# szaguldo-kamaz/FRI-ReinforcementLearning-C

Measured on AMD Instinct MI355X. Metric: rule-distance evals/sec (rules x envs), higher is better.
Workload: dtype f64; 1 GPU; cfg4_acrobot_64k_x_8k_per_gpu; nant=5, universe_len=41, rules_per_env=65536, envs_per_gpu=8192, exact_hits=4, dist_backend=none, world_size=1

## Files before the change

fri-reinforcementlearning-c_amd/__init__.py:

```python
import ctypes as C
import os

PKG_DIR = os.path.dirname(os.path.abspath(__file__))
ROOT = os.path.dirname(PKG_DIR)
HIP_LIB_PATH = os.environ.get("FRIRL_HIP_LIB_OVERRIDE") or os.path.join(PKG_DIR, "lib", "libfrirl_hip.so")

NO_HIT = 0xFFFFFFFF
MAX_NANT = 16
MAX_ACTIONS = 32


class FrirlHipError(RuntimeError):
    pass


class Tables(C.Structure):
    _fields_ = [("nant", C.c_int32), ("U", C.c_int32), ("u", C.c_void_p), ("ve", C.c_void_p)]


class RuleBases(C.Structure):
    _fields_ = [("E", C.c_int32), ("maxR", C.c_int32), ("rb", C.c_void_p), ("nrules", C.c_void_p), ("uidx", C.c_void_p)]


MAX_GRID = 64
# ... 71 lines not shown
    "frirl_hip_pack_codes": (C.c_int, [C.POINTER(Tables), C.POINTER(RuleBases), C.c_void_p, C.POINTER(C.c_int32), C.c_void_p, C.c_void_p]),
    "five_hip_rule_distance_coded_ws": (C.c_int, [C.POINTER(Tables), C.POINTER(RuleBases), C.c_void_p, C.c_void_p, C.POINTER(C.c_int32), C.c_void_p,
                                                  C.c_void_p, C.c_void_p, C.c_void_p, C.c_void_p, C.c_size_t, C.c_void_p]),
    "five_hip_sqrt_unscaled_check": (C.c_int, [C.c_void_p, C.c_void_p, C.c_void_p, C.c_int64, C.c_void_p]),
    "five_hip_rule_distance_sq_guard": (C.c_int, [C.POINTER(Tables), C.c_int32, C.c_void_p, C.c_void_p, C.c_void_p]),
    "five_hip_vag_concl": (C.c_int, [C.POINTER(Tables), C.POINTER(RuleBases), C.c_int, C.c_void_p, C.c_void_p, C.c_void_p, C.c_void_p]),
    "five_hip_vag_concl_weight": (C.c_int, [C.POINTER(Tables), C.POINTER(RuleBases), C.c_int, C.c_void_p, C.c_void_p, C.c_void_p, C.c_void_p]),
    "frirl_hip_get_best_action": (C.c_int, [C.POINTER(Tables), C.POINTER(RuleBases), C.c_int, C.c_void_p, C.c_void_p, C.c_int,
                                            C.c_void_p, C.c_void_p, C.c_void_p]),
    "five_hip_shepard_weight_check": (C.c_int, [C.c_void_p, C.c_int64, C.c_int, C.c_int, C.c_void_p, C.c_void_p]),
    "frirl_hip_explore_check": (C.c_int, [C.POINTER(AgentDesc), C.c_int64, C.c_void_p, C.c_void_p, C.c_void_p, C.c_void_p, C.c_void_p, C.c_void_p,
                                          C.c_void_p]),
    "five_hip_vag_concl_shared": (C.c_int, [C.POINTER(Tables), C.POINTER(RuleBases), C.c_int, C.c_int32, C.c_void_p, C.c_void_p, C.c_void_p, C.c_void_p]),
    "frirl_hip_get_best_action_shared": (C.c_int, [C.POINTER(Tables), C.POINTER(RuleBases), C.c_int, C.c_int32, C.c_void_p, C.c_void_p, C.c_int,
                                                   C.c_void_p, C.c_void_p, C.c_void_p]),
    "frirl_hip_rollout_shared": (C.c_int, [C.POINTER(Tables), C.POINTER(RuleBases), C.POINTER(AgentDesc), C.c_int32, C.POINTER(RolloutDesc), C.c_void_p]),
    "frirl_hip_reduce_shared": (C.c_int, [C.POINTER(Tables), C.POINTER(RuleBases), C.POINTER(AgentDesc), C.c_void_p, C.c_int, C.c_double, C.c_int,
                                          C.POINTER(C.c_int32), C.POINTER(ReduceResult), C.c_void_p]),
    "frirl_hip_lanes_preferred": (C.c_int, [C.c_int32, C.c_int32, C.c_int32]),
    "frirl_hip_lanes_workspace_bytes": (C.c_size_t, [C.c_int32, C.c_int32, C.c_int32, C.c_int32]),
    "frirl_hip_episode_run_lanes": (C.c_int, [C.POINTER(Tables), C.POINTER(RuleBases), C.POINTER(AgentDesc), C.POINTER(EnvsDesc), C.c_int32,
                                              C.c_void_p, C.c_size_t, C.c_void_p]),
    "frirl_hip_rollout_resident_rules": (C.c_int, [C.c_int32, C.c_int32, C.c_int32, C.c_int32]),
    "frirl_hip_learn_supported": (C.c_int, [C.c_int32, C.c_int32, C.c_int32, C.c_int32, C.c_int32]),
    "frirl_hip_learn_plan": (C.c_int, [C.c_int32, C.c_int32, C.POINTER(C.c_int32), C.POINTER(C.c_int32)]),
    "frirl_hip_learn_workspace_bytes": (C.c_size_t, [C.c_int32, C.c_int32, C.c_int32, C.c_int32]),
    "frirl_hip_learn_run": (C.c_int, [C.POINTER(Tables), C.POINTER(RuleBases), C.POINTER(AgentDesc), C.POINTER(EnvsDesc), C.POINTER(ConvergenceDesc),
                                      C.c_void_p, C.c_int32, C.c_int32, C.c_int32, C.c_void_p, C.c_void_p, C.c_void_p, C.c_size_t, C.c_void_p]),
    "frirl_hip_learn_train_workspace_bytes": (C.c_size_t, [C.c_int32, C.c_int32, C.c_int32, C.c_int32]),
    "frirl_hip_learn_train": (C.c_int, [C.POINTER(Tables), C.POINTER(RuleBases), C.POINTER(AgentDesc), C.POINTER(EnvsDesc), C.POINTER(ConvergenceDesc),
                                        C.c_int32, C.c_int32, C.c_void_p, C.c_void_p, C.c_void_p, C.c_void_p, C.c_size_t, C.POINTER(C.c_int32),
                                        LEARN_CHUNK_FN, C.c_void_p, C.c_void_p]),
    "five_hip_add_rule": (C.c_int, [C.POINTER(Tables), C.POINTER(RuleBases), C.c_void_p, C.c_void_p, C.c_void_p, C.c_void_p, C.c_void_p,
                                    C.c_void_p]),
    "frirl_hip_update_sarsa": (C.c_int, [C.POINTER(Tables), C.POINTER(RuleBases), C.POINTER(AgentDesc), C.POINTER(EnvsDesc), C.c_void_p,
                                         C.c_void_p, C.c_void_p, C.c_void_p, C.c_void_p]),
    "frirl_hip_env_step": (C.c_int, [C.POINTER(AgentDesc), C.c_int32, C.c_int32, C.c_void_p, C.c_void_p, C.c_void_p, C.c_void_p, C.c_void_p,
                                     C.c_void_p, C.c_void_p]),
    "frirl_hip_episode_begin": (C.c_int, [C.POINTER(Tables), C.POINTER(RuleBases), C.POINTER(AgentDesc), C.POINTER(EnvsDesc), C.c_void_p]),
    "frirl_hip_episode_step": (C.c_int, [C.POINTER(Tables), C.POINTER(RuleBases), C.POINTER(AgentDesc), C.POINTER(EnvsDesc), C.c_void_p]),
    "frirl_hip_episode_steps": (C.c_int, [C.POINTER(Tables), C.POINTER(RuleBases), C.POINTER(AgentDesc), C.POINTER(EnvsDesc), C.c_int32, C.c_void_p]),
    "frirl_hip_agent_begin": (C.c_int, [C.POINTER(Tables), C.POINTER(RuleBases), C.POINTER(AgentDesc), C.POINTER(EnvsDesc), C.POINTER(AgentIO), C.c_void_p]),
    "frirl_hip_agent_observe": (C.c_int, [C.POINTER(Tables), C.POINTER(RuleBases), C.POINTER(AgentDesc), C.POINTER(EnvsDesc), C.POINTER(AgentIO),
                                          C.c_void_p]),
    "frirl_hip_policy_begin": (C.c_int, [C.POINTER(Tables), C.POINTER(RuleBases), C.POINTER(AgentDesc), C.POINTER(PolicyRowsDesc), C.POINTER(AgentIO), C.c_void_p]),
    "frirl_hip_policy_observe": (C.c_int, [C.POINTER(Tables), C.POINTER(RuleBases), C.POINTER(AgentDesc), C.POINTER(PolicyRowsDesc), C.POINTER(AgentIO),
# ... 74 lines not shown
        for name, (res, args) in SIGNATURES.items():
            fn = getattr(L, name)
            fn.restype, fn.argtypes = res, args
        _lib = L
    return _lib


def check(rc, what=""):
    if rc != 0:
        raise FrirlHipError(f"{what}: rc={rc}: {lib().frirl_hip_last_error().decode()}")


def set_option(name, value):
    old = C.c_int()
    check(lib().frirl_hip_get_option(name.encode(), C.byref(old)), "frirl_hip_get_option")
    check(lib().frirl_hip_set_option(name.encode(), int(value)), "frirl_hip_set_option")
    return old.value


def _ptr(t):
    return None if t is None else C.c_void_p(t.data_ptr())


def _stream(stream=None):
    import torch
    s = stream if stream is not None else torch.cuda.current_stream()
    return C.c_void_p(s.cuda_stream)


class Problem:

    def __init__(self, u, ve, rb, nrules, uidx=None):
        import torch
        assert u.is_cuda and ve.is_cuda and rb.is_cuda and nrules.is_cuda
        assert u.dtype == torch.float64 and ve.dtype == torch.float64 and rb.dtype == torch.float64 and nrules.dtype == torch.int32
        self.nant, self.U = u.shape
        self.E, cols, self.maxR = rb.shape
        assert cols == self.nant + 1 and ve.shape == u.shape and nrules.shape == (self.E,)
        self.u, self.ve, self.rb, self.nrules = u.contiguous(), ve.contiguous(), rb.contiguous(), nrules.contiguous()
        self.uidx = None
        if uidx is not None:
            assert uidx.is_cuda and uidx.dtype == torch.int16 and uidx.shape == (self.E, self.nant, self.maxR) and self.U <= 32767
            self.uidx = uidx.contiguous()
        self.tables = Tables(self.nant, self.U, self.u.data_ptr(), self.ve.data_ptr())
        self._bases = RuleBases(self.E, self.maxR, self.rb.data_ptr(), self.nrules.data_ptr(),
                                self.uidx.data_ptr() if self.uidx is not None else None)
# ... 631 lines not shown
    for k in range(nant):
        idx = torch.randint(0, U, (E, R), generator=g, device=device)
        if k == nant - 1:
            idx = a_idx[torch.randint(0, A, (E, R), generator=g, device=device)]
        gk = d["grids"][k]
        lo_i, hi_i = int(np.argmin(np.abs(d["u"][k] - gk.min()))), int(np.argmin(np.abs(d["u"][k] - gk.max())))
        divider = ncorner >> (k + 1)
        corner = torch.tensor([lo_i if ((j // divider) % 2) == 0 else hi_i for j in range(ncorner)], device=device)
        idx[:, :ncorner] = corner[None]
        rb[:, k, :R] = ve_d[k][idx]
        if keep_rant:
            rant[:, k, :R] = u_d[k][idx]
        if compressed:
            uidx[:, k, :R] = idx.to(torch.int16)
        del idx
    rb[:, nant, ncorner:R] = torch.rand((E, R - ncorner), generator=g, device=device, dtype=torch.float64) * 3000.0 - 1500.0
    nrules = torch.full((E,), R, dtype=torch.int32, device=device)
    prob = Problem(u_d, ve_d, rb, nrules, uidx)
    agent = demo_agent(d, device, max_steps)
    envs = Envs(prob, device, keep_rant=keep_rant, rant_init=rant)
    return prob, agent, envs


def demo_agent(d, device, max_steps=None, p=0, **kw):
    return Agent(device, d["nant"], d["grids"], d["grid_div"], d["values_def"], d["action_ve"], d["alpha"], d["gamma"], d["qdiff_pos"],
                 d["qdiff_neg"], d["weight_thr"], d["skip_rules"], p, d["kind"], max_steps or d["max_steps"],
                 reward_good_above=d["reward_good_above"], qdiff_final_tolerance=d["qdiff_final_tolerance"], **kw)


def describe(states, actions, U, alpha, gamma, qdiff_pos, qdiff_neg, weight_thr=0.05, skip_rules=1, reward_good_above=0.0,
             qdiff_final_tolerance=250.0, max_steps=1000, name="external"):
    import numpy as np
    D = dropin()
    dims = list(states) + [dict(actions, steep=0.0, default=0.0)]
    nant = len(dims)
    assert 2 <= nant <= MAX_NANT - 1
    grid = np.zeros((nant, MAX_GRID))
    grid_len = np.zeros(nant, dtype=np.int32)
    grid_div, values_def, steep, udiv = np.zeros(nant), np.zeros(nant), np.zeros(nant), np.zeros(nant)
    for k, d in enumerate(dims):
        if d.get("values") is not None:
            v = np.asarray(d["values"], dtype=np.float64)
        else:
            v = np.zeros(int(d["n"]))
            D.frirl_gen_fixres_arr(v.ctypes.data_as(C.POINTER(C.c_double)), len(v), float(d["div"]))
        assert 1 <= len(v) <= MAX_GRID
# ... 43 lines not shown
```

fri-reinforcementlearning-c_amd/csrc/device_common.h:

```cpp
#pragma once

#include <hip/hip_runtime.h>
#include <stdint.h>

#include "../../include/frirl_hip.h"

#define FRIRL_WAVE 64
#define FRIRL_BLOCK 256
#define FRIRL_WAVES_PER_BLOCK (FRIRL_BLOCK / FRIRL_WAVE)

namespace frirl {

__device__ __forceinline__ unsigned snap_index(const double *__restrict__ uni, int len, double point, double div)
{
    const int low = (int)((point - uni[0]) / div);
    if (low < 0) return 0u;
    if (low >= len) return (unsigned)(len - 1);
    if (low + 1 >= len) return (unsigned)low;
    const double d1 = uni[low] - point;
    const double d2 = uni[low + 1] - point;
    return (fabs(d1) <= fabs(d2)) ? (unsigned)low : (unsigned)(low + 1);
}

__device__ __forceinline__ double universe_div(const double *__restrict__ uni, int U)
{
    return (uni[U - 1] - uni[0]) / (double)(U - 1);
}

__device__ __forceinline__ double observe_ve(const double *__restrict__ u, const double *__restrict__ ve, int U, int k, double xk)
{
    const double *uni = u + (size_t)k * U;
    return ve[(size_t)k * U + snap_index(uni, U, xk, universe_div(uni, U))];
}

#ifndef FRIRL_DECODE_MAD
#define FRIRL_DECODE_MAD 1
#endif
typedef __attribute__((address_space(3))) const double lds_cdouble;
__device__ __forceinline__ double2 lds_table_pair(const double *tab_k, uint32_t w)
{
    double2 v;
#if FRIRL_DECODE_MAD
    const uint32_t base = (uint32_t)(uintptr_t)(lds_cdouble *)tab_k;
    uint32_t a0, a1;
    asm("v_mad_u32_u16 %0, %1, 8, %2 op_sel:[0,0,0,0]" : "=v"(a0) : "v"(w), "s"(base));
    asm("v_mad_u32_u16 %0, %1, 8, %2 op_sel:[1,0,0,0]" : "=v"(a1) : "v"(w), "s"(base));
    v.x = *(lds_cdouble *)(uintptr_t)a0;
// ... 87 lines not shown

struct Options {
    int no_uidx;
    int rd_unroll;
    int rd_chunk;
    int rd_nt;
    int rd_persist;
    int rd_order;
    int rd_packed;
    int rd_sqdiff;
    int rd_qpass;
    int rd_prepass;
    int rd_coded;
    int step_wave;
    int step_track;
    int lanes_slices;
    int lanes_wpe;
    int rollout_group;
    int rollout_slices;
    int rollout_resident;
    int rollout_cap;
    int rollout_pair;
    int rollout_wps;
    int policy_group;
    int policy_slices;
    int learn_slices;
    int learn_alone;
    int learn_persistent;
    int multi_loopback;
    int mirror_sync;
    int no_many;
};
const Options &opts();
}
```

fri-reinforcementlearning-c_amd/csrc/rollout.hip:

```cpp
#include "sweeps.h"
#include "envs.h"
#include <mutex>
#include <type_traits>
#include <vector>

namespace frirl {

constexpr int RR_BLOCK = 256;

struct RolloutCtl {
    unsigned next[32];
    unsigned count[8];
    unsigned too_big;
    unsigned pad[7];
};

struct RolloutPark {
    int32_t *env;
    double *states;
    double *total;
    int32_t *steps;
    int32_t *act;
};

struct RolloutPhase {
    int from_parked;
    int stage;
    unsigned lo, hi;
    int cap;
    int qslot;
    int rps;
    int ht;
};

constexpr uint32_t HT_EMPTY = 0xFFFFFFFFu;

__device__ __forceinline__ uint32_t hash_mix(uint32_t hsh, double x)
// ... 455 lines not shown
            const PairSpec<NANT> &o = spec_s[buf][act_s[buf]];
#pragma unroll
            for (int k = 0; k < NS; k++) { states[k] = o.state[k]; q[k] = o.q[k]; }
            total = total + o.reward;
            success = o.success;
            steps++;
            fresh = false;
            ended = success == 1 || steps >= ag.max_steps;
        }
        if (threadIdx.x == 0) {
            ro.steps[qi] = steps;
            ro.reward[qi] = total;
            if (ro.success) ro.success[qi] = success;
            if (ro.final_states)
                for (int k = 0; k < NS; k++) ro.final_states[(size_t)qi * NS + k] = states[k];
            item_s = atomicAdd(&ctl->next[ph.qslot], 1u);
        }
        __syncthreads();
        item = (unsigned)__builtin_amdgcn_readfirstlane((int)item_s);
        __syncthreads();
    }
}

}

using namespace frirl_host;

namespace {

struct StreamWs { hipStream_t s; int dev; char *p; size_t bytes; };
std::mutex g_ws_mu;
std::vector<StreamWs> g_ws;
struct WsCleanup { ~WsCleanup() { for (StreamWs &w : g_ws) if (w.p) (void)hipFree(w.p); } } g_ws_cleanup;
char *stream_workspace(hipStream_t s, size_t bytes)
{
    int dev = 0;
    (void)hipGetDevice(&dev);
    std::lock_guard<std::mutex> lk(g_ws_mu);
    for (StreamWs &w : g_ws)
        if (w.s == s && w.dev == dev) {
            if (w.bytes >= bytes) return w.p;
            (void)hipStreamSynchronize(s);
            (void)hipFree(w.p);
            w.p = nullptr; w.bytes = 0;
            if (hipMalloc(reinterpret_cast<void **>(&w.p), bytes) != hipSuccess) { (void)hipGetLastError(); w.p = nullptr; return nullptr; }
            w.bytes = bytes;
            return w.p;
        }
    StreamWs w{s, dev, nullptr, bytes};
    if (hipMalloc(reinterpret_cast<void **>(&w.p), bytes) != hipSuccess) { (void)hipGetLastError(); return nullptr; }
    g_ws.push_back(w);
    return w.p;
}

int g_cus = 0;
int device_cus()
{
    if (g_cus) return g_cus;
    int dev = 0, n = 0;
    if (hipGetDevice(&dev) != hipSuccess || hipDeviceGetAttribute(&n, hipDeviceAttributeMultiprocessorCount, dev) != hipSuccess || n < 1) n = 256;
    g_cus = n;
    return n;
}

template <int N, int NA, int KIND, int H, bool EXCL>
void launch_phase(const frirl_hip_tables *t, const frirl_hip_rulebases *b, const frirl_hip_agent *ag, int Q, const frirl_hip_rollout *ro,
                  frirl::RolloutCtl *ctl, const frirl::RolloutPark &src, const frirl::RolloutPark &dst, const frirl::RolloutPhase &ph, unsigned items_max, int wps,
                  hipStream_t s)
{
    const size_t dyn = (size_t)(N + 1) * ph.rps * sizeof(double) + (KIND != FRIRL_HIP_ENV_CARTPOLE ? 2 * sizeof(double) * N * (size_t)t->U : 0) + sizeof(uint32_t) * (size_t)ph.ht +
                       (EXCL ? (size_t)ph.rps : 0);
    const long need = ((long)items_max * H + frirl::RR_BLOCK - 1) / frirl::RR_BLOCK;
// ... 131 lines not shown
        int H0 = 2;
        while (H0 < 64 && (long)Q * (2 * H0) <= lanes) H0 *= 2;
        if (o.rollout_slices == 2 || o.rollout_slices == 4 || o.rollout_slices == 8 || o.rollout_slices == 16 || o.rollout_slices == 32 || o.rollout_slices == 64) H0 = o.rollout_slices;
        ph.from_parked = 0; ph.stage = 0; ph.cap = nstages > 1 ? budget[0] : never;
        PHASE(H0, (unsigned)Q, list[0], list[0]);
        unsigned in_max = (unsigned)Q;
        for (int st = 1; st < nstages; st++) {
            ph.from_parked = 1; ph.stage = st; ph.cap = st == nstages - 1 ? never : budget[st];
            const frirl::RolloutPark &src = list[(st - 1) & 1], &dst = list[st & 1];
            for (int H = 64; H >= 2; H /= 2) {
                const long fit = lanes / H;
                ph.lo = H == 64 ? 0u : (unsigned)(fit / 2 < 0xffffffffL ? fit / 2 : 0xffffffffL);
                ph.hi = H == 2 ? 0xffffffffu : (unsigned)fit;
                if (ph.lo >= in_max) continue;
                PHASE(H, (unsigned)((long)in_max < fit || H == 2 ? in_max : fit), src, dst);
            }
        }
    }
#undef PHASE
    *too_big_flag = rps_full > cap_rules ? &ctl->too_big : nullptr;
    *workspace = nullptr;
    return 1;
}
```

fri-reinforcementlearning-c_amd/csrc/runtime.hip:

```cpp
#include <stdarg.h>
#include <stdio.h>
#include <stdlib.h>
#include <string.h>

#include <mutex>

#include "device_common.h"

namespace frirl_host {

static thread_local char g_err[512] = "";

void set_error(const char *fmt, ...)
{
    va_list ap;
    va_start(ap, fmt);
    vsnprintf(g_err, sizeof g_err, fmt, ap);
    va_end(ap);
}

static Options g_opts;
static std::once_flag g_opts_once;
struct OptName { const char *name, *env; int Options::*field; int def; };
static const OptName k_opts[] = {
    {"no_uidx", "FRIRL_HIP_NO_UIDX", &Options::no_uidx, 0},
    {"rd_unroll", "FRIRL_HIP_RD_UNROLL", &Options::rd_unroll, 0},
    {"rd_chunk", "FRIRL_HIP_RD_CHUNK", &Options::rd_chunk, 0},
    {"rd_nt", "FRIRL_HIP_RD_NT", &Options::rd_nt, -1},
    {"rd_persist", "FRIRL_HIP_RD_PERSIST", &Options::rd_persist, -1},
    {"rd_order", "FRIRL_HIP_RD_ORDER", &Options::rd_order, 0},
    {"rd_packed", "FRIRL_HIP_RD_PACKED", &Options::rd_packed, 1},
    {"rd_sqdiff", "FRIRL_HIP_RD_SQDIFF", &Options::rd_sqdiff, 1},
    {"rd_qpass", "FRIRL_HIP_RD_QPASS", &Options::rd_qpass, 0},
    {"rd_prepass", "FRIRL_HIP_RD_PREPASS", &Options::rd_prepass, 1},
    {"rd_coded", "FRIRL_HIP_RD_CODED", &Options::rd_coded, 1},
    {"step_wave", "FRIRL_HIP_STEP_WAVE", &Options::step_wave, -1},
    {"step_track", "FRIRL_HIP_STEP_TRACK", &Options::step_track, -1},
    {"lanes_slices", "FRIRL_HIP_LANES_SLICES", &Options::lanes_slices, 0},
    {"lanes_wpe", "FRIRL_HIP_LANES_WPE", &Options::lanes_wpe, 0},
    {"rollout_group", "FRIRL_HIP_ROLLOUT_GROUP", &Options::rollout_group, 0},
    {"rollout_slices", "FRIRL_HIP_ROLLOUT_SLICES", &Options::rollout_slices, 0},
    {"rollout_resident", "FRIRL_HIP_ROLLOUT_RESIDENT", &Options::rollout_resident, -1},
    {"rollout_cap", "FRIRL_HIP_ROLLOUT_CAP", &Options::rollout_cap, 0},
    {"rollout_pair", "FRIRL_HIP_ROLLOUT_PAIR", &Options::rollout_pair, -1},
    {"rollout_wps", "FRIRL_HIP_ROLLOUT_WPS", &Options::rollout_wps, 0},
    {"policy_group", "FRIRL_HIP_POLICY_GROUP", &Options::policy_group, 0},
    {"policy_slices", "FRIRL_HIP_POLICY_SLICES", &Options::policy_slices, 0},
    {"learn_slices", "FRIRL_HIP_LEARN_SLICES", &Options::learn_slices, 0},
    {"learn_alone", "FRIRL_HIP_LEARN_ALONE", &Options::learn_alone, 0},
    {"learn_persistent", "FRIRL_HIP_LEARN_PERSISTENT", &Options::learn_persistent, -1},
    {"multi_loopback", "FRIRL_HIP_MULTI_LOOPBACK", &Options::multi_loopback, 0},
    {"no_many", "FRIRL_HIP_NO_MANY", &Options::no_many, 0},
    {"mirror_sync", "FRIRL_HIP_MIRROR_SYNC", &Options::mirror_sync, 0},
};
static void opts_init()
{
    for (const OptName &o : k_opts) {
        const char *e = getenv(o.env);
        g_opts.*(o.field) = e ? atoi(e) : o.def;
    }
}
const Options &opts()
{
    std::call_once(g_opts_once, opts_init);
    return g_opts;
}
static const OptName *find_opt(const char *name)
{
// ... 104 lines not shown
```

fri-reinforcementlearning-c_amd/csrc/shared.hip:

```cpp
#include "shared_sweep.h"
#include "envs.h"
#include "reduce_plan.h"
#include <algorithm>
#include <cstdlib>
#include <cstring>
#include <cmath>
#include <numeric>
#include <vector>

namespace frirl {

template <int NANT, int AMAX, bool GBA>
__global__ __launch_bounds__(SH_BLOCK) void shared_q_kernel(const double *__restrict__ u, const double *__restrict__ ve, int U,
                                                             const double *__restrict__ rb, const int32_t *__restrict__ nrules, int maxR, int p,
                                                             int Q, const double *__restrict__ x, const double *__restrict__ action_ve, int A,
                                                             double *__restrict__ conc, uint32_t *__restrict__ hit, int32_t *__restrict__ best)
{
    constexpr int ND = GBA ? NANT - 1 : NANT;
    __shared__ SharedTile<NANT> tl;
    const int qi = blockIdx.x * SH_BLOCK + threadIdx.x;
    const bool live = qi < Q;
    double q[ND];
#pragma unroll
    for (int k = 0; k < ND; k++) q[k] = live ? observe_ve(u, ve, U, k, x[(size_t)qi * ND + k]) : 0.0;
    if (GBA && (int)threadIdx.x < A) tl.ave[threadIdx.x] = action_ve[threadIdx.x];
    unsigned h0;
    int bi;
    double bv;
    shared_sweep<NANT, AMAX, GBA, false>(tl, rb, nullptr, nrules[0], maxR, PowU{p}, 0, A, GBA ? (A + AMAX - 1) / AMAX : 1, q, live, 0u,
                                         live ? conc + (size_t)qi * (GBA ? A : 1) : nullptr, h0, bi, bv);
    if (!live) return;
    if (GBA) best[qi] = bi;
    else hit[qi] = h0;
}

template <int NANT, int AMAX, int G, int H, bool EXCL, bool PN = true>
__global__ __launch_bounds__(SH_BLOCK) void rollout_shared_kernel(const double *__restrict__ u, const double *__restrict__ ve, int U,
                                                                   const double *__restrict__ rb, const int32_t *__restrict__ nrules, int maxR,
                                                                   const frirl_hip_agent ag, int Q, const frirl_hip_rollout ro,
                                                                   const unsigned *__restrict__ run_if)
{
    constexpr int NS = NANT - 1, GH = G * H, EPB = SH_BLOCK / GH;
    if (run_if && *run_if == 0u) return;
    __shared__ SharedTile<NANT> tl;
    __shared__ double grid_s[NANT * FRIRL_HIP_MAX_GRID];
    const int gl = threadIdx.x % GH, sub = gl % G, h = gl / G;
    const int qi = blockIdx.x * EPB + threadIdx.x / GH;
    const bool exists = qi < Q;
    const int R = nrules[0];
    using POW = typename std::conditional<PN, PowC<NANT>, PowU>::type;
    POW p;
    if constexpr (!PN) p.p = ag.p > 0 ? ag.p : NANT;
    const int apl = (ag.A + G - 1) / G;
// ... 76 lines not shown
        set_error("%s: env_kind %d does not match nant=%d (the demo environments only)", who, agent->env_kind, t->nant);
        return FRIRL_HIP_EINVAL;
    }
    return FRIRL_HIP_OK;
}

extern "C" int five_hip_vag_concl_shared(const frirl_hip_tables *t, const frirl_hip_rulebases *b, int p, int32_t Q, const double *x,
                                         double *conc, uint32_t *hit, void *stream)
{
    int rc = check_shared(t, b, Q, "five_hip_vag_concl_shared");
    if (rc) return rc;
    if (!x || !conc || !hit) { set_error("five_hip_vag_concl_shared: NULL argument"); return FRIRL_HIP_EINVAL; }
    const int pp = p > 0 ? p : t->nant;
    const dim3 grid((Q + frirl::SH_BLOCK - 1) / frirl::SH_BLOCK);
    switch (t->nant) {
#define M(N) case N: hipLaunchKernelGGL((frirl::shared_q_kernel<N, 1, false>), grid, dim3(frirl::SH_BLOCK), 0, as_stream(stream), t->u, t->ve, t->U, b->rb, \
                                        b->nrules, b->maxR, pp, Q, x, nullptr, 1, conc, hit, nullptr); break;
        M(2) M(3) M(4) M(5) M(6) M(7) M(8) M(9)
#undef M
    }
    return check_launch("five_hip_vag_concl_shared");
}

extern "C" int frirl_hip_get_best_action_shared(const frirl_hip_tables *t, const frirl_hip_rulebases *b, int p, int32_t Q, const double *states,
                                                const double *action_ve, int A, double *actconc, int32_t *best, void *stream)
{
    int rc = check_shared(t, b, Q, "frirl_hip_get_best_action_shared");
    if (rc) return rc;
    if (!states || !action_ve || !actconc || !best || A < 1 || A > FRIRL_HIP_MAX_ACTIONS) { set_error("frirl_hip_get_best_action_shared: bad arguments"); return FRIRL_HIP_EINVAL; }
    const int pp = p > 0 ? p : t->nant;
    const dim3 grid((Q + frirl::SH_BLOCK - 1) / frirl::SH_BLOCK);
    switch (t->nant) {
#define M(N)                                                                                                                                              \
    case N:                                                                                                                                               \
        if (A <= 4) hipLaunchKernelGGL((frirl::shared_q_kernel<N, 4, true>), grid, dim3(frirl::SH_BLOCK), 0, as_stream(stream), t->u, t->ve, t->U, b->rb,   \
                                       b->nrules, b->maxR, pp, Q, states, action_ve, A, actconc, nullptr, best);                                          \
        else hipLaunchKernelGGL((frirl::shared_q_kernel<N, 8, true>), grid, dim3(frirl::SH_BLOCK), 0, as_stream(stream), t->u, t->ve, t->U, b->rb,         \
                                b->nrules, b->maxR, pp, Q, states, action_ve, A, actconc, nullptr, best);                                                 \
        break;
        M(2) M(3) M(4) M(5) M(6) M(7) M(8) M(9)
#undef M
    }
    return check_launch("frirl_hip_get_best_action_shared");
}

template <int N, int AMAX, int G, int H, bool PN = true>
static void launch_rollout(const frirl_hip_tables *t, const frirl_hip_rulebases *b, const frirl_hip_agent *ag, int Q, const frirl_hip_rollout *ro,
                           hipStream_t s, const unsigned *run_if)
{
    constexpr int EPB = frirl::SH_BLOCK / (G * H);
    const dim3 grid((Q + EPB - 1) / EPB);
    if (ro->exclude_mask && ro->rule_slot)
        hipLaunchKernelGGL((frirl::rollout_shared_kernel<N, AMAX, G, H, true, PN>), grid, dim3(frirl::SH_BLOCK), 0, s, t->u, t->ve, t->U, b->rb, b->nrules, b->maxR, *ag, Q, *ro, run_if);
    else
        hipLaunchKernelGGL((frirl::rollout_shared_kernel<N, AMAX, G, H, false, PN>), grid, dim3(frirl::SH_BLOCK), 0, s, t->u, t->ve, t->U, b->rb, b->nrules, b->maxR, *ag, Q, *ro, run_if);
}

static int rollout_group(int Q, int A)
{
    { const int g = frirl_host::opts().rollout_group; if (g == 1 || (g == 4 && A <= 4) || (g == 8 && A > 4)) return g; }
    if (A < 2 || Q >= 131072) return 1;
    return A <= 4 ? 4 : 8;
}

static int rollout_slices(int Q, int G)
// ... 14 lines not shown
    else launch_rollout<N, AMAX, G, 1>(t, b, ag, Q, ro, s, run_if);
}

template <int N>
static void launch_rollout_n(const frirl_hip_tables *t, const frirl_hip_rulebases *b, const frirl_hip_agent *ag, int Q, const frirl_hip_rollout *ro,
                             hipStream_t s, const unsigned *run_if)
{
    const int G = rollout_group(Q, ag->A);
    if (ag->p > 0 && ag->p != N) {
        if (G == 4) launch_rollout<N, 1, 4, 1, false>(t, b, ag, Q, ro, s, run_if);
        else if (G == 8) launch_rollout<N, 4, 8, 1, false>(t, b, ag, Q, ro, s, run_if);
        else if (ag->A <= 4) launch_rollout<N, 4, 1, 1, false>(t, b, ag, Q, ro, s, run_if);
        else launch_rollout<N, 8, 1, 1, false>(t, b, ag, Q, ro, s, run_if);
        return;
    }
    if (G == 4) launch_rollout_h<N, 1, 4>(t, b, ag, Q, ro, s, run_if);
    else if (G == 8) launch_rollout_h<N, 4, 8>(t, b, ag, Q, ro, s, run_if);
    else if (ag->A <= 4) launch_rollout<N, 4, 1, 1>(t, b, ag, Q, ro, s, run_if);
    else launch_rollout<N, 8, 1, 1>(t, b, ag, Q, ro, s, run_if);
}

int frirl_rollout_resident(const frirl_hip_tables *t, const frirl_hip_rulebases *b, const frirl_hip_agent *ag, int Q, const frirl_hip_rollout *ro,
                           hipStream_t s, const unsigned **too_big_flag, void **workspace);

extern "C" int frirl_hip_rollout_shared(const frirl_hip_tables *t, const frirl_hip_rulebases *b, const frirl_hip_agent *agent, int32_t Q,
                                        const frirl_hip_rollout *ro, void *stream)
{
    int rc = check_shared_args(t, b, Q, "frirl_hip_rollout_shared");
    if (rc) return rc;
    if (!agent || !ro || !ro->steps || !ro->reward || !agent->grid_values || !agent->action_ve) { set_error("frirl_hip_rollout_shared: NULL argument"); return FRIRL_HIP_EINVAL; }
    if (agent->A < 1 || agent->A > FRIRL_HIP_MAX_ACTIONS || agent->max_steps < 0) { set_error("frirl_hip_rollout_shared: A=%d / max_steps=%d out of range", agent->A, agent->max_steps); return FRIRL_HIP_EINVAL; }
    for (int k = 0; k < t->nant; k++)
        if (agent->grid_len[k] < 1 || agent->grid_len[k] > FRIRL_HIP_MAX_GRID) { set_error("frirl_hip_rollout_shared: grid_len[%d]=%d outside 1..%d", k, agent->grid_len[k], FRIRL_HIP_MAX_GRID); return FRIRL_HIP_EINVAL; }
    if ((ro->exclude_mask == nullptr) != (ro->rule_slot == nullptr)) { set_error("frirl_hip_rollout_shared: exclude_mask and rule_slot go together"); return FRIRL_HIP_EINVAL; }
    if ((rc = check_demo_kind(t, agent, "frirl_hip_rollout_shared")) || (rc = check_device())) return rc;
    hipStream_t s = as_stream(stream);
    const unsigned *too_big = nullptr;
    void *ws = nullptr;
    if (frirl_rollout_resident(t, b, agent, Q, ro, s, &too_big, &ws)) {
        if (too_big) {
            if (t->nant == 3) launch_rollout_n<3>(t, b, agent, Q, ro, s, too_big);
            else launch_rollout_n<5>(t, b, agent, Q, ro, s, too_big);
        }
        if (ws) (void)hipFreeAsync(ws, s);
        return check_launch("frirl_hip_rollout_shared");
    }
    if (t->nant == 3) launch_rollout_n<3>(t, b, agent, Q, ro, s, nullptr);
    else launch_rollout_n<5>(t, b, agent, Q, ro, s, nullptr);
    return check_launch("frirl_hip_rollout_shared");
}

namespace {
struct DevBuf {
    void *p = nullptr;
    ~DevBuf() { if (p) (void)hipFree(p); }
    bool alloc(size_t n) { return hipMalloc(&p, n ? n : 1) == hipSuccess; }
};
}

// ... 58 lines not shown
```

include/frirl_hip.h:

```cpp
#ifndef FRIRL_HIP_H
#define FRIRL_HIP_H

#include <stdint.h>

#ifdef __cplusplus
extern "C" {
#endif

#define FRIRL_HIP_MAX_NANT     16
#define FRIRL_HIP_MAX_ACTIONS  32
#define FRIRL_HIP_MAX_GRID     64
#define FRIRL_HIP_NO_HIT       0xFFFFFFFFu

#define FRIRL_HIP_ENV_MOUNTAINCAR 0
#define FRIRL_HIP_ENV_CARTPOLE    1
#define FRIRL_HIP_ENV_ACROBOT     2
#define FRIRL_HIP_ENV_EXTERNAL    3

#define FRIRL_HIP_UPD_INACTIVE   0
#define FRIRL_HIP_UPD_EXACT      1
#define FRIRL_HIP_UPD_SPREAD     2
#define FRIRL_HIP_UPD_INSERTED   3
#define FRIRL_HIP_UPD_SKIPPED    4
#define FRIRL_HIP_UPD_FULL       5
// ... 79 lines not shown
    double qdiff_final_tolerance;
    uint64_t seed;
    int32_t evaluate;
    int32_t debug_flags;
    uint64_t env_id_base;
} frirl_hip_agent;

int frirl_hip_explore_check(const frirl_hip_agent *agent, int64_t n, const uint32_t *env, const uint32_t *episode, const uint32_t *step,
                            const int32_t *greedy, int32_t *out_action, double *out_unit, void *stream);

typedef struct frirl_hip_rollout {
    const double *start_states;
    const uint32_t *exclude_mask;
    const uint8_t *rule_slot;
    int32_t *steps;
    double *reward;
    int32_t *success;
    double *final_states;
} frirl_hip_rollout;
int frirl_hip_rollout_shared(const frirl_hip_tables *t, const frirl_hip_rulebases *b, const frirl_hip_agent *agent, int32_t Q,
                             const frirl_hip_rollout *ro, void *stream);
int frirl_hip_rollout_resident_rules(int32_t nant, int32_t A, int32_t p, int32_t env_kind);

typedef struct frirl_hip_reduce_result {
    int32_t rules_before, rules_after;
    int32_t rounds;
    int32_t rollouts;
    int32_t steps_incremental;
    int32_t reserved;
    double reward;
} frirl_hip_reduce_result;
int frirl_hip_reduce_shared(const frirl_hip_tables *t, const frirl_hip_rulebases *b, const frirl_hip_agent *agent, double *rant, int strategy,
                            double reward_tolerance, int depth, int32_t *kept, frirl_hip_reduce_result *result, void *stream);

typedef struct frirl_hip_envs {
    double *states;
    double *q_ant;
    int32_t *fus;
    int32_t *done;
    int32_t *ep_steps;
    double *ep_reward;
    double *rant;
    int32_t *status;
    const double *start_states;
    int32_t *episode;
    double *spread_ant;
// ... 186 lines not shown
```

Before: 545.7 billion evals/s.

## Precompute greedy action table over quantized grid cells for rollouts

```diff
diff --git a/fri-reinforcementlearning-c_amd/__init__.py b/fri-reinforcementlearning-c_amd/__init__.py
--- a/fri-reinforcementlearning-c_amd/__init__.py
+++ b/fri-reinforcementlearning-c_amd/__init__.py
@@ -117,6 +117,9 @@
     "frirl_hip_episode_run_lanes": (C.c_int, [C.POINTER(Tables), C.POINTER(RuleBases), C.POINTER(AgentDesc), C.POINTER(EnvsDesc), C.c_int32,
                                               C.c_void_p, C.c_size_t, C.c_void_p]),
     "frirl_hip_rollout_resident_rules": (C.c_int, [C.c_int32, C.c_int32, C.c_int32, C.c_int32]),
+    "frirl_hip_rollout_table_cells": (C.c_int, [C.POINTER(Tables), C.POINTER(AgentDesc), C.c_int32, C.POINTER(C.c_int32), C.c_void_p, C.POINTER(C.c_int32)]),
+    "frirl_hip_rollout_table_stats": (C.c_int, [C.c_void_p, C.POINTER(C.c_uint32), C.POINTER(C.c_uint32)]),
+    "frirl_hip_rollout_table_read": (C.c_int, [C.c_void_p, C.c_int32, C.POINTER(C.c_int32)]),
     "frirl_hip_learn_supported": (C.c_int, [C.c_int32, C.c_int32, C.c_int32, C.c_int32, C.c_int32]),
     "frirl_hip_learn_plan": (C.c_int, [C.c_int32, C.c_int32, C.POINTER(C.c_int32), C.POINTER(C.c_int32)]),
     "frirl_hip_learn_workspace_bytes": (C.c_size_t, [C.c_int32, C.c_int32, C.c_int32, C.c_int32]),
@@ -237,6 +240,21 @@
     return None if t is None else C.c_void_p(t.data_ptr())
 
 
+def rollout_table_stats(stream=None):
+    ran, misses = C.c_uint32(), C.c_uint32()
+    check(lib().frirl_hip_rollout_table_stats(_stream(stream), C.byref(ran), C.byref(misses)), "frirl_hip_rollout_table_stats")
+    return ran.value, misses.value
+
+
+def rollout_table_read(stream=None):
+    import numpy as np
+    table = np.zeros(4096, dtype=np.int32)
+    n = lib().frirl_hip_rollout_table_read(_stream(stream), table.size, table.ctypes.data_as(C.POINTER(C.c_int32)))
+    if n < 0:
+        check(n, "frirl_hip_rollout_table_read")
+    return table[:n].copy()
+
+
 def _stream(stream=None):
     import torch
     s = stream if stream is not None else torch.cuda.current_stream()
@@ -914,6 +932,26 @@
     return prob, agent, envs
 
 
+def rollout_table_cells(d, holes=0):
+    import numpy as np
+    nant, U = d["nant"], d["U"]
+    u = np.ascontiguousarray(d["u"], dtype=np.float64)
+    grid = np.zeros((nant, MAX_GRID))
+    desc = AgentDesc()
+    desc.env_kind, desc.A = d["kind"], d["A"]
+    for k in range(nant):
+        grid[k, : len(d["grids"][k])] = d["grids"][k]
+        desc.grid_len[k] = len(d["grids"][k])
+    desc.grid_values = grid.ctypes.data
+    tables = Tables(nant, U, u.ctypes.data, u.ctypes.data)
+    nrank = np.zeros(nant - 1, dtype=np.int32)
+    rank = np.zeros((nant - 1, U), dtype=np.uint8)
+    cells = C.c_int32()
+    check(lib().frirl_hip_rollout_table_cells(C.byref(tables), C.byref(desc), int(holes), nrank.ctypes.data_as(C.POINTER(C.c_int32)),
+                                              C.c_void_p(rank.ctypes.data), C.byref(cells)), "frirl_hip_rollout_table_cells")
+    return cells.value, nrank, rank
+
+
 def demo_agent(d, device, max_steps=None, p=0, **kw):
     return Agent(device, d["nant"], d["grids"], d["grid_div"], d["values_def"], d["action_ve"], d["alpha"], d["gamma"], d["qdiff_pos"],
                  d["qdiff_neg"], d["weight_thr"], d["skip_rules"], p, d["kind"], max_steps or d["max_steps"],
diff --git a/fri-reinforcementlearning-c_amd/csrc/device_common.h b/fri-reinforcementlearning-c_amd/csrc/device_common.h
--- a/fri-reinforcementlearning-c_amd/csrc/device_common.h
+++ b/fri-reinforcementlearning-c_amd/csrc/device_common.h
@@ -11,7 +11,7 @@
 
 namespace frirl {
 
-__device__ __forceinline__ unsigned snap_index(const double *__restrict__ uni, int len, double point, double div)
+__host__ __device__ __forceinline__ unsigned snap_index(const double *__restrict__ uni, int len, double point, double div)
 {
     const int low = (int)((point - uni[0]) / div);
     if (low < 0) return 0u;
@@ -22,7 +22,7 @@
     return (fabs(d1) <= fabs(d2)) ? (unsigned)low : (unsigned)(low + 1);
 }
 
-__device__ __forceinline__ double universe_div(const double *__restrict__ uni, int U)
+__host__ __device__ __forceinline__ double universe_div(const double *__restrict__ uni, int U)
 {
     return (uni[U - 1] - uni[0]) / (double)(U - 1);
 }
@@ -156,6 +156,8 @@
     int rollout_cap;
     int rollout_pair;
     int rollout_wps;
+    int rollout_table;
+    int rollout_table_holes;
     int policy_group;
     int policy_slices;
     int learn_slices;
diff --git a/fri-reinforcementlearning-c_amd/csrc/rollout.hip b/fri-reinforcementlearning-c_amd/csrc/rollout.hip
--- a/fri-reinforcementlearning-c_amd/csrc/rollout.hip
+++ b/fri-reinforcementlearning-c_amd/csrc/rollout.hip
@@ -1,5 +1,6 @@
 #include "sweeps.h"
 #include "envs.h"
+#include <algorithm>
 #include <mutex>
 #include <type_traits>
 #include <vector>
@@ -12,7 +13,9 @@
     unsigned next[32];
     unsigned count[8];
     unsigned too_big;
-    unsigned pad[7];
+    unsigned table_ran;
+    unsigned table_misses;
+    unsigned pad[5];
 };
 
 struct RolloutPark {
@@ -514,13 +517,198 @@
     }
 }
 
+constexpr int RT_BLOCK = 256;
+constexpr int RT_MAX_CELLS = 4096;
+
+struct TableShape { int len[FRIRL_HIP_MAX_NANT]; };
+
+__host__ __device__ inline double table_candidate(int kind, const double *grid, int k, int j)
+{
+    if (kind == FRIRL_HIP_ENV_CARTPOLE) {
+        if (k != 2) return (double)(j - 1);
+        const double deg12 = FRIRL_PI / 15, deg3 = FRIRL_PI / 60;
+        if (j < 9) return (double)(j - 4) * deg3;
+        return j == 9 ? -1 * deg12 : deg12;
+    }
+    return grid[(size_t)k * FRIRL_HIP_MAX_GRID + j];
+}
+
+__host__ __device__ inline int table_list_len(int kind, const int32_t *grid_len, int k)
+{
+    return kind == FRIRL_HIP_ENV_CARTPOLE ? (k == 2 ? 11 : 3) : grid_len[k];
+}
+
+__host__ __device__ inline int table_rank_row(int kind, const double *uni, int U, const double *grid, int k, int len, bool skip_last, uint8_t *rank_k)
+{
+    const double div = universe_div(uni, U);
+    int n = 0;
+    for (int j = 0; j < len; j++) {
+        const unsigned idx = snap_index(uni, U, table_candidate(kind, grid, k, j), div);
+        if (rank_k[idx] != 255) continue;
+        n++;
+        if (!(skip_last && j == len - 1)) rank_k[idx] = (uint8_t)j;
+    }
+    return n;
+}
+
+__global__ __launch_bounds__(RT_BLOCK) void table_setup_kernel(const double *__restrict__ u, int U, const frirl_hip_agent ag, int NS, const TableShape sh, int ncells,
+                                                               int holes, uint8_t *__restrict__ rank_g, double *__restrict__ rows_g)
+{
+    for (int i = threadIdx.x; i < NS * U; i += RT_BLOCK) rank_g[i] = 255;
+    __syncthreads();
+    if ((int)threadIdx.x < NS) {
+        const int k = threadIdx.x;
+        (void)table_rank_row(ag.env_kind, u + (size_t)k * U, U, ag.grid_values, k, sh.len[k], holes && k == 0, rank_g + (size_t)k * U);
+    }
+    for (int c = threadIdx.x; c <= ncells; c += RT_BLOCK) {
+        int rest = c;
+        for (int k = NS - 1; k >= 0; k--) {
+            const int j = rest % sh.len[k];
+            rest /= sh.len[k];
+            rows_g[(size_t)c * NS + k] = c < ncells ? table_candidate(ag.env_kind, ag.grid_values, k, j) : ag.values_def[k];
+        }
+    }
+}
+
+template <int NANT, int KIND>
+__global__ __launch_bounds__(RT_BLOCK) void rollout_table_kernel(const double *__restrict__ u, const double *__restrict__ ve, int U,
+                                                                 const double *__restrict__ rb, const int32_t *__restrict__ nrules, int maxR,
+                                                                 const frirl_hip_agent ag, int Q, const frirl_hip_rollout ro, RolloutCtl *__restrict__ ctl,
+                                                                 const TableShape sh, int ncells, const uint8_t *__restrict__ rank_g,
+                                                                 const int32_t *__restrict__ best_g)
+{
+    constexpr int NS = NANT - 1;
+    constexpr bool LT = KIND != FRIRL_HIP_ENV_CARTPOLE;
+    extern __shared__ __attribute__((aligned(16))) double dyn_s[];
+    __shared__ uint8_t table_s[RT_MAX_CELLS];
+    __shared__ double grid_s[NANT * FRIRL_HIP_MAX_GRID];
+    uint8_t *rank_s = reinterpret_cast<uint8_t *>(dyn_s + (LT ? NS * U : 0));
+    for (int i = threadIdx.x; i < ncells; i += RT_BLOCK) table_s[i] = (uint8_t)best_g[i];
+    for (int i = threadIdx.x; i < NS * U; i += RT_BLOCK) rank_s[i] = rank_g[i];
+    if (LT) for (int i = threadIdx.x; i < NS * U; i += RT_BLOCK) dyn_s[i] = u[i];
+    for (int i = threadIdx.x; i < NANT * FRIRL_HIP_MAX_GRID; i += RT_BLOCK) grid_s[i] = ag.grid_values[i];
+    if (blockIdx.x == 0 && threadIdx.x == 0) ctl->table_ran = 1u;
+    __syncthreads();
+    const double *us;
+    if constexpr (LT) us = dyn_s; else us = u;
+    double udiv[NS];
+#pragma unroll
+    for (int k = 0; k < NS; k++) udiv[k] = universe_div(us + (size_t)k * U, U);
+    const int32_t *first_g = best_g + ncells;
+    const int R = nrules[0];
+    const int lane = threadIdx.x & (FRIRL_WAVE - 1);
+
+    double states[NS], cur[NS], total = 0.0, action = 0.0;
+    int qi = 0, steps = 0, success = 0;
+    bool active = false, fresh = false, drained = false;
+#pragma unroll
+    for (int k = 0; k < NS; k++) { states[k] = 0.0; cur[k] = 0.0; }
+
+    for (;;) {
+        const bool want = !active && !drained;
+        const unsigned long long wb = __ballot(want);
+        if (wb) {
+            const int first = __ffsll((long long)wb) - 1;
+            unsigned base = 0u;
+            if (lane == first) base = atomicAdd(&ctl->next[0], (unsigned)__popcll(wb));
+            base = (unsigned)__shfl((int)base, first);
+            const unsigned item = base + (unsigned)__popcll(wb & ((1ull << lane) - 1ull));
+            if (want) {
+                if (item < (unsigned)Q) {
+                    active = true;
+                    fresh = true;
+                    success = 0;
+                    qi = (int)item;
+                    steps = 0;
+                    total = 0.0;
+#pragma unroll
+                    for (int k = 0; k < NS; k++) states[k] = ro.start_states ? ro.start_states[(size_t)qi * NS + k] : ag.values_def[k];
+                } else {
+                    drained = true;
+                }
+            }
+        }
+        if (!__any(active ? 1 : 0)) break;
+
+        if (active) {
+            int pa;
+            bool ended = false;
+            if (fresh) {
+                pa = first_g[ro.start_states ? 1 + qi : 0];
+                pa = e_greedy(ag, pa, (uint32_t)qi, 0u, 0u);
+                fresh = false;
+            } else {
+                double r, qs[NS];
+                env_do_action(KIND, action, states, cur);
+                env_get_reward(KIND, cur, r, success);
+                total = total + r;
+                env_quantize(KIND, NS, grid_s, ag.grid_len, ag.grid_div, cur, qs);
+                unsigned idx[NS];
+                int cell = 0;
+                bool miss = false;
+#pragma unroll
+                for (int k = 0; k < NS; k++) {
+                    idx[k] = snap_index(us + (size_t)k * U, U, qs[k], udiv[k]);
+                    const int rk = rank_s[k * U + idx[k]];
+                    miss = miss || rk == 255;
+                    cell = cell * sh.len[k] + rk;
+                }
+                if (!miss) {
+                    pa = table_s[cell];
+                } else {
+                    atomicAdd(&ctl->table_misses, 1u);
+                    const PowU pk{ag.p > 0 ? ag.p : NANT};
+                    double q[NS], bv = 0.0;
+#pragma unroll
+                    for (int k = 0; k < NS; k++) q[k] = ve[(size_t)k * U + idx[k]];
+                    pa = 0;
+                    for (int a = 0; a < ag.A; a++) {
+                        const double av = ag.action_ve[a];
+                        double sv = 0.0, sw = 0.0;
+                        unsigned hit = FRIRL_HIP_NO_HIT;
+                        for (int rr = 0; rr < R; rr++) {
+                            const double d0 = q[0] - rb[rr];
+                            double s = d0 * d0;
+#pragma unroll
+                            for (int k = 1; k < NS; k++) { const double d = q[k] - rb[(size_t)k * maxR + rr]; s = __fma_rn(d, d, s); }
+                            const double e = av - rb[(size_t)NS * maxR + rr];
+                            const double d2 = __fma_rn(e, e, s);
+                            const double wi = shepard_w(d2, pk);
+                            sv = __fma_rn(wi, rb[(size_t)NANT * maxR + rr], sv);
+                            sw = sw + wi;
+                            hit = (d2 == 0.0 && hit == FRIRL_HIP_NO_HIT) ? (unsigned)rr : hit;
+                        }
+                        const double c = (hit != FRIRL_HIP_NO_HIT) ? rb[(size_t)NANT * maxR + hit] : sv / sw;
+                        if (a == 0 || bv < c) { bv = c; pa = a; }
+                    }
+                }
+                pa = e_greedy(ag, pa, (uint32_t)qi, 0u, (uint32_t)(steps + 1));
+#pragma unroll
+                for (int k = 0; k < NS; k++) states[k] = cur[k];
+                steps++;
+                if (success == 1) ended = true;
+            }
+            action = grid_s[NS * FRIRL_HIP_MAX_GRID + pa];
+            if (!ended && steps >= ag.max_steps) ended = true;
+            if (ended) {
+                active = false;
+                ro.steps[qi] = steps;
+                ro.reward[qi] = total;
+                if (ro.success) ro.success[qi] = success;
+                if (ro.final_states)
+                    for (int k = 0; k < NS; k++) ro.final_states[(size_t)qi * NS + k] = states[k];
+            }
+        }
+    }
+}
+
 }
 
 using namespace frirl_host;
 
 namespace {
 
-struct StreamWs { hipStream_t s; int dev; char *p; size_t bytes; };
+struct StreamWs { hipStream_t s; int dev; char *p; size_t bytes; size_t table_off; int table_n; };
 std::mutex g_ws_mu;
 std::vector<StreamWs> g_ws;
 struct WsCleanup { ~WsCleanup() { for (StreamWs &w : g_ws) if (w.p) (void)hipFree(w.p); } } g_ws_cleanup;
@@ -539,7 +727,7 @@
             w.bytes = bytes;
             return w.p;
         }
-    StreamWs w{s, dev, nullptr, bytes};
+    StreamWs w{s, dev, nullptr, bytes, 0, 0};
     if (hipMalloc(reinterpret_cast<void **>(&w.p), bytes) != hipSuccess) { (void)hipGetLastError(); return nullptr; }
     g_ws.push_back(w);
     return w.p;
@@ -717,3 +905,142 @@
     *workspace = nullptr;
     return 1;
 }
+
+void frirl_launch_best_action_shared(const frirl_hip_tables *t, const frirl_hip_rulebases *b, int p, int32_t Q, const double *states, const double *action_ve,
+                                     int A, double *actconc, int32_t *best, hipStream_t s);
+
+static int table_shape(const frirl_hip_tables *t, const frirl_hip_agent *ag, frirl::TableShape *sh)
+{
+    const int NS = t->nant - 1;
+    long cells = 1;
+    for (int k = 0; k < NS; k++) {
+        const int len = frirl::table_list_len(ag->env_kind, ag->grid_len, k);
+        if (len < 1 || len > 64) return 0;
+        sh->len[k] = len;
+        cells *= len;
+        if (cells > frirl::RT_MAX_CELLS) return 0;
+    }
+    return (int)cells;
+}
+
+extern "C" int frirl_hip_rollout_table_cells(const frirl_hip_tables *t, const frirl_hip_agent *agent, int32_t holes, int32_t *nrank, uint8_t *rank, int32_t *cells)
+{
+    int rc = check_tables(t);
+    if (rc) return rc;
+    if (!agent || !agent->grid_values || !nrank || !cells) { set_error("frirl_hip_rollout_table_cells: NULL argument"); return FRIRL_HIP_EINVAL; }
+    if (agent->env_kind < 0 || agent->env_kind > 2 || (agent->env_kind == FRIRL_HIP_ENV_MOUNTAINCAR ? t->nant != 3 : t->nant != 5)) {
+        set_error("frirl_hip_rollout_table_cells: env_kind %d does not match nant=%d", agent->env_kind, t->nant);
+        return FRIRL_HIP_EINVAL;
+    }
+    frirl::TableShape sh = {};
+    *cells = 0;
+    if (!table_shape(t, agent, &sh)) return FRIRL_HIP_OK;
+    const int NS = t->nant - 1;
+    std::vector<uint8_t> row((size_t)t->U);
+    long n = 1;
+    for (int k = 0; k < NS; k++) {
+        std::fill(row.begin(), row.end(), (uint8_t)255);
+        nrank[k] = frirl::table_rank_row(agent->env_kind, t->u + (size_t)k * t->U, t->U, agent->grid_values, k, sh.len[k], holes && k == 0, row.data());
+        if (rank) std::copy(row.begin(), row.end(), rank + (size_t)k * t->U);
+        n *= nrank[k];
+    }
+    *cells = (int32_t)n;
+    return FRIRL_HIP_OK;
+}
+
+extern "C" int frirl_hip_rollout_table_stats(void *stream, uint32_t *ran, uint32_t *misses)
+{
+    if (!ran || !misses) { set_error("frirl_hip_rollout_table_stats: NULL argument"); return FRIRL_HIP_EINVAL; }
+    *ran = *misses = 0u;
+    int rc = check_device();
+    if (rc) return rc;
+    hipStream_t s = as_stream(stream);
+    int dev = 0;
+    (void)hipGetDevice(&dev);
+    const char *ws = nullptr;
+    {
+        std::lock_guard<std::mutex> lk(g_ws_mu);
+        for (const StreamWs &w : g_ws) if (w.s == s && w.dev == dev && w.table_n > 0) ws = w.p;
+    }
+    if (!ws) return FRIRL_HIP_OK;
+    frirl::RolloutCtl ctl;
+    if (hipStreamSynchronize(s) != hipSuccess || hipMemcpy(&ctl, ws, sizeof ctl, hipMemcpyDeviceToHost) != hipSuccess) {
+        set_error("frirl_hip_rollout_table_stats: %s", hipGetErrorString(hipGetLastError()));
+        return FRIRL_HIP_ELAUNCH;
+    }
+    *ran = ctl.table_ran;
+    *misses = ctl.table_misses;
+    return FRIRL_HIP_OK;
+}
+
+extern "C" int frirl_hip_rollout_table_read(void *stream, int32_t n, int32_t *table)
+{
+    if (n < 0 || (n > 0 && !table)) { set_error("frirl_hip_rollout_table_read: bad arguments"); return FRIRL_HIP_EINVAL; }
+    uint32_t ran = 0, misses = 0;
+    int rc = frirl_hip_rollout_table_stats(stream, &ran, &misses);
+    if (rc) return rc;
+    if (!ran) return 0;
+    hipStream_t s = as_stream(stream);
+    int dev = 0;
+    (void)hipGetDevice(&dev);
+    const char *src = nullptr;
+    int have = 0;
+    {
+        std::lock_guard<std::mutex> lk(g_ws_mu);
+        for (const StreamWs &w : g_ws) if (w.s == s && w.dev == dev) { src = w.p + w.table_off; have = w.table_n; }
+    }
+    const int m = n < have ? n : have;
+    if (m > 0 && hipMemcpy(table, src, sizeof(int32_t) * (size_t)m, hipMemcpyDeviceToHost) != hipSuccess) {
+        set_error("frirl_hip_rollout_table_read: %s", hipGetErrorString(hipGetLastError()));
+        return FRIRL_HIP_ELAUNCH;
+    }
+    return have;
+}
+
+void frirl_rollout_table_forget(hipStream_t s)
+{
+    int dev = 0;
+    (void)hipGetDevice(&dev);
+    std::lock_guard<std::mutex> lk(g_ws_mu);
+    for (StreamWs &w : g_ws) if (w.s == s && w.dev == dev) w.table_n = 0;
+}
+
+int frirl_rollout_table(const frirl_hip_tables *t, const frirl_hip_rulebases *b, const frirl_hip_agent *ag, int Q, const frirl_hip_rollout *ro, hipStream_t s)
+{
+    frirl::TableShape sh = {};
+    const int ncells = table_shape(t, ag, &sh);
+    if (!ncells) return 0;
+    const int NS = t->nant - 1;
+    const bool lt = ag->env_kind != FRIRL_HIP_ENV_CARTPOLE;
+    const size_t rank_bytes = ((size_t)NS * t->U + 63) / 64 * 64;
+    const size_t dyn = (lt ? sizeof(double) * NS * (size_t)t->U : 0) + rank_bytes;
+    if (dyn > 32 * 1024) return 0;
+    const size_t ctl_bytes = (sizeof(frirl::RolloutCtl) + 63) / 64 * 64;
+    const size_t rows_bytes = (sizeof(double) * (size_t)(ncells + 1) * NS + 63) / 64 * 64;
+    const size_t nfirst = ro->start_states ? (size_t)Q : 0;
+    char *ws = stream_workspace(s, ctl_bytes + rank_bytes + rows_bytes + sizeof(int32_t) * ((size_t)ncells + 1 + nfirst));
+    if (!ws) return 0;
+    (void)hipMemsetAsync(ws, 0, ctl_bytes, s);
+    frirl::RolloutCtl *ctl = reinterpret_cast<frirl::RolloutCtl *>(ws);
+    uint8_t *rank_g = reinterpret_cast<uint8_t *>(ws + ctl_bytes);
+    double *rows_g = reinterpret_cast<double *>(ws + ctl_bytes + rank_bytes);
+    int32_t *best_g = reinterpret_cast<int32_t *>(ws + ctl_bytes + rank_bytes + rows_bytes);
+    {
+        int dev = 0;
+        (void)hipGetDevice(&dev);
+        std::lock_guard<std::mutex> lk(g_ws_mu);
+        for (StreamWs &w : g_ws) if (w.s == s && w.dev == dev) { w.table_off = ctl_bytes + rank_bytes + rows_bytes; w.table_n = ncells; }
+    }
+    hipLaunchKernelGGL(frirl::table_setup_kernel, dim3(1), dim3(frirl::RT_BLOCK), 0, s, t->u, t->U, *ag, NS, sh, ncells, opts().rollout_table_holes == 1 ? 1 : 0, rank_g, rows_g);
+    frirl_launch_best_action_shared(t, b, ag->p, ncells + 1, rows_g, ag->action_ve, ag->A, nullptr, best_g, s);
+    if (ro->start_states) frirl_launch_best_action_shared(t, b, ag->p, Q, ro->start_states, ag->action_ve, ag->A, nullptr, best_g + ncells + 1, s);
+    const long need = ((long)Q + frirl::RT_BLOCK - 1) / frirl::RT_BLOCK;
+    const long cap = 8L * device_cus();
+    const dim3 grid((unsigned)(need < cap ? need : cap));
+#define GO(N, KIND) hipLaunchKernelGGL((frirl::rollout_table_kernel<N, KIND>), grid, dim3(frirl::RT_BLOCK), dyn, s, t->u, t->ve, t->U, b->rb, b->nrules, b->maxR, *ag, Q, *ro, ctl, sh, ncells, rank_g, best_g)
+    if (ag->env_kind == FRIRL_HIP_ENV_MOUNTAINCAR) GO(3, FRIRL_HIP_ENV_MOUNTAINCAR);
+    else if (ag->env_kind == FRIRL_HIP_ENV_CARTPOLE) GO(5, FRIRL_HIP_ENV_CARTPOLE);
+    else GO(5, FRIRL_HIP_ENV_ACROBOT);
+#undef GO
+    return 1;
+}
diff --git a/fri-reinforcementlearning-c_amd/csrc/runtime.hip b/fri-reinforcementlearning-c_amd/csrc/runtime.hip
--- a/fri-reinforcementlearning-c_amd/csrc/runtime.hip
+++ b/fri-reinforcementlearning-c_amd/csrc/runtime.hip
@@ -44,6 +44,8 @@
     {"rollout_cap", "FRIRL_HIP_ROLLOUT_CAP", &Options::rollout_cap, 0},
     {"rollout_pair", "FRIRL_HIP_ROLLOUT_PAIR", &Options::rollout_pair, -1},
     {"rollout_wps", "FRIRL_HIP_ROLLOUT_WPS", &Options::rollout_wps, 0},
+    {"rollout_table", "FRIRL_HIP_ROLLOUT_TABLE", &Options::rollout_table, 1},
+    {"rollout_table_holes", "FRIRL_HIP_ROLLOUT_TABLE_HOLES", &Options::rollout_table_holes, 0},
     {"policy_group", "FRIRL_HIP_POLICY_GROUP", &Options::policy_group, 0},
     {"policy_slices", "FRIRL_HIP_POLICY_SLICES", &Options::policy_slices, 0},
     {"learn_slices", "FRIRL_HIP_LEARN_SLICES", &Options::learn_slices, 0},
diff --git a/fri-reinforcementlearning-c_amd/csrc/shared.hip b/fri-reinforcementlearning-c_amd/csrc/shared.hip
--- a/fri-reinforcementlearning-c_amd/csrc/shared.hip
+++ b/fri-reinforcementlearning-c_amd/csrc/shared.hip
@@ -28,7 +28,7 @@
     int bi;
     double bv;
     shared_sweep<NANT, AMAX, GBA, false>(tl, rb, nullptr, nrules[0], maxR, PowU{p}, 0, A, GBA ? (A + AMAX - 1) / AMAX : 1, q, live, 0u,
-                                         live ? conc + (size_t)qi * (GBA ? A : 1) : nullptr, h0, bi, bv);
+                                         (live && conc) ? conc + (size_t)qi * (GBA ? A : 1) : nullptr, h0, bi, bv);
     if (!live) return;
     if (GBA) best[qi] = bi;
     else hit[qi] = h0;
@@ -151,25 +151,31 @@
     return check_launch("five_hip_vag_concl_shared");
 }
 
-extern "C" int frirl_hip_get_best_action_shared(const frirl_hip_tables *t, const frirl_hip_rulebases *b, int p, int32_t Q, const double *states,
-                                                const double *action_ve, int A, double *actconc, int32_t *best, void *stream)
-{
-    int rc = check_shared(t, b, Q, "frirl_hip_get_best_action_shared");
-    if (rc) return rc;
-    if (!states || !action_ve || !actconc || !best || A < 1 || A > FRIRL_HIP_MAX_ACTIONS) { set_error("frirl_hip_get_best_action_shared: bad arguments"); return FRIRL_HIP_EINVAL; }
+void frirl_launch_best_action_shared(const frirl_hip_tables *t, const frirl_hip_rulebases *b, int p, int32_t Q, const double *states, const double *action_ve,
+                                     int A, double *actconc, int32_t *best, hipStream_t s)
+{
     const int pp = p > 0 ? p : t->nant;
     const dim3 grid((Q + frirl::SH_BLOCK - 1) / frirl::SH_BLOCK);
     switch (t->nant) {
 #define M(N)                                                                                                                                              \
     case N:                                                                                                                                               \
-        if (A <= 4) hipLaunchKernelGGL((frirl::shared_q_kernel<N, 4, true>), grid, dim3(frirl::SH_BLOCK), 0, as_stream(stream), t->u, t->ve, t->U, b->rb,   \
+        if (A <= 4) hipLaunchKernelGGL((frirl::shared_q_kernel<N, 4, true>), grid, dim3(frirl::SH_BLOCK), 0, s, t->u, t->ve, t->U, b->rb,   \
                                        b->nrules, b->maxR, pp, Q, states, action_ve, A, actconc, nullptr, best);                                          \
-        else hipLaunchKernelGGL((frirl::shared_q_kernel<N, 8, true>), grid, dim3(frirl::SH_BLOCK), 0, as_stream(stream), t->u, t->ve, t->U, b->rb,         \
+        else hipLaunchKernelGGL((frirl::shared_q_kernel<N, 8, true>), grid, dim3(frirl::SH_BLOCK), 0, s, t->u, t->ve, t->U, b->rb,         \
                                 b->nrules, b->maxR, pp, Q, states, action_ve, A, actconc, nullptr, best);                                                 \
         break;
         M(2) M(3) M(4) M(5) M(6) M(7) M(8) M(9)
 #undef M
     }
+}
+
+extern "C" int frirl_hip_get_best_action_shared(const frirl_hip_tables *t, const frirl_hip_rulebases *b, int p, int32_t Q, const double *states,
+                                                const double *action_ve, int A, double *actconc, int32_t *best, void *stream)
+{
+    int rc = check_shared(t, b, Q, "frirl_hip_get_best_action_shared");
+    if (rc) return rc;
+    if (!states || !action_ve || !actconc || !best || A < 1 || A > FRIRL_HIP_MAX_ACTIONS) { set_error("frirl_hip_get_best_action_shared: bad arguments"); return FRIRL_HIP_EINVAL; }
+    frirl_launch_best_action_shared(t, b, p, Q, states, action_ve, A, actconc, best, as_stream(stream));
     return check_launch("frirl_hip_get_best_action_shared");
 }
 
@@ -230,6 +236,9 @@
 
 int frirl_rollout_resident(const frirl_hip_tables *t, const frirl_hip_rulebases *b, const frirl_hip_agent *ag, int Q, const frirl_hip_rollout *ro,
                            hipStream_t s, const unsigned **too_big_flag, void **workspace);
+int frirl_rollout_table(const frirl_hip_tables *t, const frirl_hip_rulebases *b, const frirl_hip_agent *ag, int Q, const frirl_hip_rollout *ro,
+                        hipStream_t s);
+void frirl_rollout_table_forget(hipStream_t s);
 
 extern "C" int frirl_hip_rollout_shared(const frirl_hip_tables *t, const frirl_hip_rulebases *b, const frirl_hip_agent *agent, int32_t Q,
                                         const frirl_hip_rollout *ro, void *stream)
@@ -243,6 +252,14 @@
     if ((ro->exclude_mask == nullptr) != (ro->rule_slot == nullptr)) { set_error("frirl_hip_rollout_shared: exclude_mask and rule_slot go together"); return FRIRL_HIP_EINVAL; }
     if ((rc = check_demo_kind(t, agent, "frirl_hip_rollout_shared")) || (rc = check_device())) return rc;
     hipStream_t s = as_stream(stream);
+    {
+        const Options &o = opts();
+        const bool forced = o.rollout_resident != -1 || o.rollout_pair != -1 || o.rollout_slices != 0 || o.rollout_group != 0 || o.rollout_wps != 0 ||
+                            o.rollout_cap != 0;
+        if (o.rollout_table != 0 && !forced && !ro->exclude_mask && frirl_rollout_table(t, b, agent, Q, ro, s))
+            return check_launch("frirl_hip_rollout_shared");
+        frirl_rollout_table_forget(s);
+    }
     const unsigned *too_big = nullptr;
     void *ws = nullptr;
     if (frirl_rollout_resident(t, b, agent, Q, ro, s, &too_big, &ws)) {
diff --git a/include/frirl_hip.h b/include/frirl_hip.h
--- a/include/frirl_hip.h
+++ b/include/frirl_hip.h
@@ -125,6 +125,10 @@
                              const frirl_hip_rollout *ro, void *stream);
 int frirl_hip_rollout_resident_rules(int32_t nant, int32_t A, int32_t p, int32_t env_kind);
 
+int frirl_hip_rollout_table_cells(const frirl_hip_tables *t, const frirl_hip_agent *agent, int32_t holes, int32_t *nrank, uint8_t *rank, int32_t *cells);
+int frirl_hip_rollout_table_stats(void *stream, uint32_t *ran, uint32_t *misses);
+int frirl_hip_rollout_table_read(void *stream, int32_t n, int32_t *table);
+
 typedef struct frirl_hip_reduce_result {
     int32_t rules_before, rules_after;
     int32_t rounds;
```

Result: slower. 521.2 billion evals/s (-4.5%).
